# wliverno/GauNEGF

Measured on AMD Instinct MI355X. Metric: energy-points/sec (complex128 G(E) solves), higher is better.
Workload: dtype f64 (complex128)

## Files before the change

gaunegf_amd/csrc/chain_rs_inverse.h:

```cpp
#pragma once
#include "negf_common.h"
#include "wave_utils.h"

namespace {

constexpr int RS_THREADS = 256;
constexpr int RS_WAVES = 4;
#ifndef RS_PANEL
#define RS_PANEL 8
#endif
constexpr int RS_NB = RS_PANEL;
#ifndef RS_PRIO
#define RS_PRIO 1
#endif
#ifndef RS_REMAINDER
#define RS_REMAINDER 1
#endif
#ifndef RS_ROW_MODE
#define RS_ROW_MODE 0
#endif
#ifndef RS_LA_FLAGS
#define RS_LA_FLAGS 0
#endif
#ifndef RS_RR
#define RS_RR 1
#endif
#ifndef RS_UPD_3M
#define RS_UPD_3M 1
#endif
#ifndef RS_HALF_STRIPS
#define RS_HALF_STRIPS 1
#endif
#ifndef RS_ABLATE
#define RS_ABLATE 0
#endif
#ifndef RS_STAMPS
#define RS_STAMPS 0
#endif

template <int CTRL, int ROW_MASK = 0xF>
__device__ __forceinline__ unsigned rs_dpp_max_u32(unsigned k)
{
    const unsigned o = (unsigned)__builtin_amdgcn_update_dpp(0, (int)k, CTRL, ROW_MASK, 0xF, true);
    return o > k ? o : k;
}

__device__ __forceinline__ unsigned rs_wave_max_u32(unsigned k)
{
    k = rs_dpp_max_u32<0xB1>(k);
    k = rs_dpp_max_u32<0x4E>(k);
    k = rs_dpp_max_u32<0x141>(k);
    k = rs_dpp_max_u32<0x140>(k);
    k = rs_dpp_max_u32<0x142, 0xA>(k);
    k = rs_dpp_max_u32<0x143, 0xC>(k);
    return (unsigned)__builtin_amdgcn_readlane((int)k, 63);
}

__device__ __forceinline__ void zmfma4(double& ar, double& ai, cplx pa, cplx qb)
{
    ar = __builtin_amdgcn_mfma_f64_4x4x4f64(pa.x, qb.x, ar, 0, 0, 0);
    ar = __builtin_amdgcn_mfma_f64_4x4x4f64(pa.y, -qb.y, ar, 0, 0, 0);
    ai = __builtin_amdgcn_mfma_f64_4x4x4f64(pa.x, qb.y, ai, 0, 0, 0);
    ai = __builtin_amdgcn_mfma_f64_4x4x4f64(pa.y, qb.x, ai, 0, 0, 0);
}
__device__ __forceinline__ void zmfma4_conjb(double& ar, double& ai, cplx pa, cplx b)
{
    ar = __builtin_amdgcn_mfma_f64_4x4x4f64(pa.x, b.x, ar, 0, 0, 0);
// ... 4 lines not shown
#define RS_M3S(A, B, C, PR, PI, PS, QR, QI, QS) do { double a_ = (A)[0], b_ = (B)[0], c_ = (C)[0]; mfma3s(a_, b_, c_, PR, PI, PS, QR, QI, QS); (A)[0] = a_; (B)[0] = b_; (C)[0] = c_; } while (0)
#define RS_ZMFMA4(ACCR, ACCI, PA, QB) do { double r_ = (ACCR)[0], i_ = (ACCI)[0]; zmfma4(r_, i_, PA, QB); (ACCR)[0] = r_; (ACCI)[0] = i_; } while (0)
#define RS_ZMFMA4C(ACCR, ACCI, PA, QB) do { double r_ = (ACCR)[0], i_ = (ACCI)[0]; zmfma4_conjb(r_, i_, PA, QB); (ACCR)[0] = r_; (ACCI)[0] = i_; } while (0)

__device__ __forceinline__ void mfma3(d4& a, d4& b, d4& c, double pr, double pi, double ps, double qr, double qi, double qs)
{
    a = __builtin_amdgcn_mfma_f64_16x16x4f64(pr, qr, a, 0, 0, 0);
    b = __builtin_amdgcn_mfma_f64_16x16x4f64(pi, qi, b, 0, 0, 0);
    c = __builtin_amdgcn_mfma_f64_16x16x4f64(ps, qs, c, 0, 0, 0);
}
#ifndef RS_3M_GEMM
#define RS_3M_GEMM 1
#endif
__device__ __forceinline__ void mfma3s(double& a, double& b, double& c, double pr, double pi, double ps, double qr, double qi, double qs)
{
    a = __builtin_amdgcn_mfma_f64_4x4x4f64(pr, qr, a, 0, 0, 0);
    b = __builtin_amdgcn_mfma_f64_4x4x4f64(pi, qi, b, 0, 0, 0);
    c = __builtin_amdgcn_mfma_f64_4x4x4f64(ps, qs, c, 0, 0, 0);
}

template <class T>
__device__ __forceinline__ T rs_opaque(T v)
{
    asm volatile("" : "+v"(v));
    return v;
}

__device__ __forceinline__ double rs_readlane_f64(double v, int srclane)
{
    return __hiloint2double(__builtin_amdgcn_readlane(__double2hiint(v), srclane),
                            __builtin_amdgcn_readlane(__double2loint(v), srclane));
}

template <int P>
__device__ __forceinline__ void rs_factor(int n, cplx* W, int* pivrow, int* colof, cplx* rowline ,
                                          int p0, int pw, int lane, unsigned long long* fst = nullptr )
{
    const int r = rs_opaque(lane);
    cplx a[RS_NB];
    bool avail = r < n && colof[r] < 0;
    cplx myip = cmake(1.0, 0.0);
    cplx* wrow = W + r * P + p0;
#pragma unroll
    for (int s = 0; s < RS_NB; ++s) {
        const cplx v = wrow[s];
        const bool ok = (r < n) & (s < pw);
        a[s] = cmake(ok ? v.x : 0.0, ok ? v.y : 0.0);
    }
#pragma unroll
    for (int j = 0; j < RS_NB; ++j) {
        if (j < pw) {
            const bool stamp_here = fst && j == 4;
            unsigned long long tq0 = 0, tq1 = 0, tq2 = 0, tq3 = 0, tq4 = 0;
            if (stamp_here) tq0 = __builtin_amdgcn_s_memtime();
            const double v = cabs1(a[j]);
            const unsigned hi = (avail && v == v) ? (unsigned)__double2hiint(v) : 0u;
            const unsigned m = rs_wave_max_u32(hi);
            int pphys;
            if (m != 0) {
                pphys = (int)__ffsll((unsigned long long)__ballot(hi == m)) - 1;
            } else {
                const unsigned long long av = __ballot(avail);
                pphys = av ? (int)__ffsll(av) - 1 : 0x7fffffff;
            }
            pphys = __builtin_amdgcn_readfirstlane(pphys);
            if (stamp_here) tq1 = __builtin_amdgcn_s_memtime();
            const bool is_piv = r == pphys;
            cplx rb[RS_NB];
#if RS_ROW_MODE == 0
            __builtin_amdgcn_wave_barrier();
            if (is_piv) {
                pivrow[p0 + j] = pphys; colof[pphys] = p0 + j;
#pragma unroll
                for (int s = 0; s < RS_NB; ++s) rowline[s] = a[s];
            }
            __builtin_amdgcn_fence(__ATOMIC_RELEASE, "wavefront");
            __builtin_amdgcn_wave_barrier();
            __builtin_amdgcn_fence(__ATOMIC_ACQUIRE, "wavefront");
#pragma unroll
            for (int s = 0; s < RS_NB; ++s) rb[s] = rowline[s];
#elif RS_ROW_MODE == 1
            if (is_piv) { pivrow[p0 + j] = pphys; colof[pphys] = p0 + j; }
#pragma unroll
            for (int s = 0; s < RS_NB; ++s)
                rb[s] = cmake(rs_readlane_f64(a[s].x, pphys), rs_readlane_f64(a[s].y, pphys));
#else
            if (is_piv) { pivrow[p0 + j] = pphys; colof[pphys] = p0 + j; }
            const int baddr = pphys << 2;
#pragma unroll
            for (int s = 0; s < RS_NB; ++s) {
                rb[s].x = __hiloint2double(__builtin_amdgcn_ds_bpermute(baddr, __double2hiint(a[s].x)),
                                           __builtin_amdgcn_ds_bpermute(baddr, __double2loint(a[s].x)));
                rb[s].y = __hiloint2double(__builtin_amdgcn_ds_bpermute(baddr, __double2hiint(a[s].y)),
                                           __builtin_amdgcn_ds_bpermute(baddr, __double2loint(a[s].y)));
            }
#endif
            if (stamp_here) { asm volatile("s_waitcnt lgkmcnt(0)" ::: "memory"); tq2 = __builtin_amdgcn_s_memtime(); }
            const cplx pv = rb[j];
            const double d = pv.x * pv.x + pv.y * pv.y;
            double sc = __builtin_amdgcn_rcp(d);
            sc = fma(sc, fma(-d, sc, 1.0), sc);
            sc = fma(sc, fma(-d, sc, 1.0), sc);
            const cplx ip = cmake(pv.x * sc, -pv.y * sc);
            const cplx mf = cneg(cmul(a[j], ip));
            const cplx coef = cmake(is_piv ? 0.0 : mf.x, is_piv ? 0.0 : mf.y);
            if (stamp_here) { asm volatile("" :: "v"(coef.x), "v"(coef.y)); tq3 = __builtin_amdgcn_s_memtime(); }
#pragma unroll
            for (int s = 0; s < RS_NB; ++s) a[s] = cfma(a[s], coef, rb[s]);
            if (stamp_here) {
#pragma unroll
                for (int s = 0; s < RS_NB; ++s) asm volatile("" :: "v"(a[s].x), "v"(a[s].y));
                tq4 = __builtin_amdgcn_s_memtime();
                if (lane == 0) { fst[0] = tq0; fst[1] = tq1; fst[2] = tq2; fst[3] = tq3; fst[4] = tq4; }
            }
            a[j] = is_piv ? cmake(1.0, 0.0) : coef;
            myip = cmake(is_piv ? ip.x : myip.x, is_piv ? ip.y : myip.y);
            avail = avail && !is_piv;
        }
    }
    if (r < n) {
#pragma unroll
        for (int s = 0; s < RS_NB; ++s)
            if (s < pw) {
                wrow[s] = cmul(a[s], myip);
            }
    }
}

template <int P, int NKS, int TR >
__device__ __forceinline__ void rs_load_qf(const cplx* W, const int* pivrow, int tj, int p0, int pw, int fi, int fk,
                                           cplx (&qf)[NKS])
{
    const int col = (TR >= 0 && tj == TR) ? TR * 16 + (fi & 3) : tj * 16 + fi;
#pragma unroll
    for (int ks = 0; ks < NKS; ++ks) {
        const int k = ks * 4 + fk;
        const cplx v = W[pivrow[p0 + k] * P + col];
        const bool ok = k < pw;
        qf[ks] = cmake(ok ? v.x : 0.0, ok ? v.y : 0.0);
    }
}

__device__ __forceinline__ void rs_wait_count(const unsigned* cnt, unsigned target)
{
    while (*reinterpret_cast<const volatile unsigned*>(cnt) < target) __builtin_amdgcn_s_sleep(1);
}

template <int P, int NKS, int TR>
__device__ __forceinline__ void rs_zero_pivot_rows(int n, cplx* W, const int* pivrow, int tj, int p0, int pw, int fi, int fk,
                                                   int clo, int chi)
{
    const int col = (TR >= 0 && tj == TR) ? TR * 16 + (fi & 3) : tj * 16 + fi;
    if (col >= clo && col < chi && col < n) {
#pragma unroll
        for (int ks = 0; ks < NKS; ++ks) {
            const int k = ks * 4 + fk;
            if (k < pw) W[pivrow[p0 + k] * P + col] = cmake(0.0, 0.0);
        }
    }
}

template <int P, int NKS, int TR, bool MASK >
__device__ __forceinline__ void rs_update_tile(int n, cplx* W, const int* colof, int ti, int tj, int p0, int pw,
                                               int fi, int fk, const cplx (&qf)[NKS], int clo, int chi ,
                                               const unsigned* wait_cnt = nullptr, unsigned wait_target = 0 )
{
    const bool rowstrip = TR >= 0 && ti == TR, colstrip = TR >= 0 && tj == TR;
    if (!rowstrip && !colstrip) {
        cplx* cbase = W + (ti * 16 + fk) * P + tj * 16 + fi;
        const cplx* pbase = W + (ti * 16 + fi) * P + p0 + fk;
        cplx cv[4], pa[NKS];
// ... 14 lines not shown
            if (M3) mfma3(ua, ub, uc, pa[ks].x, pa[ks].y, pa[ks].x + pa[ks].y, qf[ks].x, qf[ks].y, qf[ks].x + qf[ks].y);
            else zmfma(ua, uc, pa[ks], qf[ks]);
        }
        if (wait_cnt) rs_wait_count(wait_cnt, wait_target);
#pragma unroll
        for (int r = 0; r < 4; ++r) {
            const int i = ti * 16 + fk + 4 * r;
            const int cj = tj * 16 + fi;
            if (i < n && cj < n && cj >= clo && cj < chi) cbase[4 * r * P] = M3 ? cmake(ua[r] - ub[r], uc[r] - ua[r] - ub[r]) : cmake(ua[r], uc[r]);
        }
    } else {
        const int row = rowstrip ? TR * 16 + fk : ti * 16 + 4 * (fi >> 2) + fk;
        const int col = colstrip ? TR * 16 + (fi & 3) : tj * 16 + fi;
        const bool mine = !(rowstrip && colstrip) || (fi >> 2) == 0;
        const cplx* prow = W + (rowstrip ? TR * 16 + (fi & 3) : ti * 16 + fi) * P + p0 + fk;
        cplx* cptr = W + row * P + col;
        const int cf = MASK ? colof[row] : -1;
        const cplx cv = *cptr;
        cplx pa[NKS];
#pragma unroll
        for (int ks = 0; ks < NKS; ++ks) pa[ks] = prow[ks * 4];
        const bool keep = !MASK || !(cf >= p0 && cf < p0 + pw);
        double ua = keep ? cv.x : 0.0, ub = 0.0, uc = keep ? cv.x + cv.y : 0.0;
#pragma unroll
        for (int ks = 0; ks < NKS; ++ks)
            mfma3s(ua, ub, uc, pa[ks].x, pa[ks].y, pa[ks].x + pa[ks].y, qf[ks].x, qf[ks].y, qf[ks].x + qf[ks].y);
        if (wait_cnt) rs_wait_count(wait_cnt, wait_target);
        if (mine && row < n && col < n && col >= clo && col < chi) *cptr = cmake(ua - ub, uc - ua - ub);
    }
}

constexpr bool rs_half_strips(int nks) { return RS_HALF_STRIPS && RS_NB == 8 && nks == RS_NB / 4; }

template <int P, int NKS>
__device__ __forceinline__ void rs_load_qh(const cplx* W, const int* pivrow, int c0, int p0, int pw, int fi, int fk,
                                           cplx (&qh)[2][NKS])
{
    const int col = c0 + (fi & 3);
#pragma unroll
    for (int ks = 0; ks < NKS; ++ks) {
        const int k = ks * 4 + fk;
        const cplx* q = W + pivrow[p0 + k] * P + col;
        const cplx v0 = q[0], v1 = q[4];
        const bool ok = k < pw;
        qh[0][ks] = cmake(ok ? v0.x : 0.0, ok ? v0.y : 0.0);
        qh[1][ks] = cmake(ok ? v1.x : 0.0, ok ? v1.y : 0.0);
    }
}

template <int P, int NKS>
__device__ __forceinline__ void rs_half_mma(cplx (&cv)[2], const cplx (&pa)[NKS], const cplx (&qh)[2][NKS], const double (&qs)[2][NKS])
{
    constexpr bool M3 = RS_UPD_3M && P > 35;
    if (M3) {
        double ua[2], ub[2] = {0.0, 0.0}, uc[2];
#pragma unroll
        for (int s = 0; s < 2; ++s) { ua[s] = cv[s].x; uc[s] = cv[s].x + cv[s].y; }
#pragma unroll
        for (int ks = 0; ks < NKS; ++ks) {
            const double ps = pa[ks].x + pa[ks].y;
#pragma unroll
            for (int s = 0; s < 2; ++s) mfma3s(ua[s], ub[s], uc[s], pa[ks].x, pa[ks].y, ps, qh[s][ks].x, qh[s][ks].y, qs[s][ks]);
        }
#pragma unroll
        for (int s = 0; s < 2; ++s) cv[s] = cmake(ua[s] - ub[s], uc[s] - ua[s] - ub[s]);
    } else {
#pragma unroll
        for (int ks = 0; ks < NKS; ++ks)
#pragma unroll
            for (int s = 0; s < 2; ++s) zmfma4(cv[s].x, cv[s].y, pa[ks], qh[s][ks]);
    }
}

template <int P, int NKS, bool FULLROWS , bool MASK>
__device__ __forceinline__ void rs_update_half(int n, cplx* W, const int* colof, int ti, int p0, int pw, int fi, int fk,
                                               const cplx (&qh)[2][NKS], int c0)
{
// ... 140 lines not shown
#pragma unroll 1
            for (int tj = 0; tj < ntiles; ++tj) {
                int clo = tj * 16, chi = tj * 16 + 16;
                if (tj == tp) {
                    if (RS_NB == 16) continue;
                    if (p0 & 8) chi = p0; else clo = p0 + RS_NB;
                }
                if (has_next && tj == tl) {
                    if (RS_NB == 16) continue;
                    if (n0 & 8) chi = min(chi, n0); else clo = max(clo, n0 + RS_NB);
                }
                if (clo >= chi || clo >= n) continue;
                const bool mine = (!has_next || wave != fw) && (cnt % team == me);
                ++cnt;
                if (mine && !(RS_ABLATE & 2)) {
                    if (pw <= 4) rs_update_col<T16, P, 1, TR>(n, W, pivrow, colof, tj, p0, pw, lane, clo, chi);
                    else rs_update_col<T16, P, RS_NB / 4, TR>(n, W, pivrow, colof, tj, p0, pw, lane, clo, chi);
                }
            }
        }
        if (has_next && wave == fw) {
            if (st && lane == 0) st[16 + 2 * (sgi + 1)] = __builtin_amdgcn_s_memrealtime();
            if (RS_PRIO) __builtin_amdgcn_s_setprio(3);
            if (!(RS_ABLATE & 1)) rs_factor<P>(n, W, pivrow, colof, rowline, n0, nw, lane, (st && sgi + 1 == 1) ? st + 40 : nullptr);
            else if (lane < nw) { pivrow[n0 + lane] = n0 + lane; colof[n0 + lane] = n0 + lane; }
            if (RS_PRIO) __builtin_amdgcn_s_setprio(0);
            if (st && lane == 0) st[17 + 2 * (sgi + 1)] = __builtin_amdgcn_s_memrealtime();
        }
        stamp();
        __syncthreads();
    }
}

}
```

gaunegf_amd/csrc/k_chain1d_rs.hip:

```cpp
#include "negf_common.h"
#include "chain_mix_map.h"
#include "chain_rs_inverse.h"
#include <algorithm>
#include <type_traits>

#ifndef RS_PAD_LEADS
#define RS_PAD_LEADS 1
#endif
#ifndef RS_BATCH_MSTORE
#define RS_BATCH_MSTORE 1
#endif
#ifndef RS_MSTORE_AHEAD
#define RS_MSTORE_AHEAD 0
#endif
#ifndef RS_DENSE_MIX
#define RS_DENSE_MIX 1
#endif

namespace {

struct ChainRsArgs {
    const cplx *alpha, *Salpha, *beta, *Sbeta, *tau, *Stau;
    const cplx* pad;
    const int* nc;
// ... 53 lines not shown
    if (i == 0) { q->head = 0u; q->tail = jobs; q->jobs = jobs; q->cap = cap; }
}

__device__ __forceinline__ double rs_uniform(double v)
{
    return __hiloint2double(__builtin_amdgcn_readfirstlane(__double2hiint(v)), __builtin_amdgcn_readfirstlane(__double2loint(v)));
}
typedef double rs_d2 __attribute__((ext_vector_type(2)));
__device__ __forceinline__ unsigned long long rs_scalar_base(const void* p)
{
    unsigned long long b = reinterpret_cast<unsigned long long>(p);
    asm volatile("" : "+s"(b));
    return b;
}
__device__ __forceinline__ unsigned long long rs_scalar_advance(unsigned long long b, long long bytes)
{
    b += (unsigned long long)bytes;
    asm volatile("" : "+s"(b));
    return b;
}
__device__ __forceinline__ cplx rs_gload(unsigned long long base, unsigned const_bytes, unsigned lane_bytes)
{
    const __attribute__((address_space(1))) char* p = reinterpret_cast<const __attribute__((address_space(1))) char*>(base) + const_bytes;
    const rs_d2 v = *reinterpret_cast<const __attribute__((address_space(1))) rs_d2*>(p + lane_bytes);
    return cmake(v.x, v.y);
}
__device__ __forceinline__ void rs_gstore(unsigned long long base, unsigned const_bytes, unsigned lane_bytes, cplx v)
{
    __attribute__((address_space(1))) char* p = reinterpret_cast<__attribute__((address_space(1))) char*>(base) + const_bytes;
    rs_d2 w; w.x = v.x; w.y = v.y;
    *reinterpret_cast<__attribute__((address_space(1))) rs_d2*>(p + lane_bytes) = w;
}

template <int P, int OCC, bool GOLD_GLOBAL, bool RR>
__global__ __launch_bounds__(RS_THREADS, OCC) void chain1d_rs_kernel(
    ChainRsArgs a, const cplx* __restrict__ E, cplx* __restrict__ blk, int* __restrict__ iters,
    int* __restrict__ converged)
{
    constexpr int T16 = (P - 1 + 15) / 16;
    constexpr int KS = (P + 3) / 4 < 4 * T16 ? (P + 3) / 4 : 4 * T16;
    constexpr int WELEMS = 16 * T16 * P + 16;
    constexpr int TR = T16 - 1;
    constexpr bool REM = RS_REMAINDER && T16 >= 2 && P - 16 * TR <= 4;
    constexpr int FT = REM ? TR : T16;
    constexpr bool M3G = T16 >= 3;
    extern __shared__ __attribute__((aligned(16))) unsigned char smem_raw[];
    __shared__ int flags[2 * RS_WAVES];
    __shared__ int pivrow[64], colof[64];
    __shared__ cplx rowline[RS_NB];
    __shared__ unsigned la_cnt[2];
    unsigned la_epoch = 0;
    if (threadIdx.x == 0) { la_cnt[0] = 0u; la_cnt[1] = 0u; }

    const int slot = blockIdx.y * gridDim.x + blockIdx.x;
    constexpr bool rr = RS_RR && RR;
    __shared__ long long rr_msg;
    cplx* Ws = reinterpret_cast<cplx*>(smem_raw);
    const int tid = threadIdx.x, lane = tid & 63;
    int wave = tid >> 6;
    bool chain_roles = false;
    if (a.simd_roles) {
        unsigned hwid;
        asm volatile("s_getreg_b32 %0, hwreg(HW_REG_HW_ID)" : "=s"(hwid));
        const int simd = (hwid >> 4) & 3;
        if (lane == 0) flags[wave] = simd;
        __syncthreads();
        const int seen = (1 << flags[0]) | (1 << flags[1]) | (1 << flags[2]) | (1 << flags[3]);
        chain_roles = __builtin_amdgcn_readfirstlane(seen) == 15;
        if (chain_roles) wave = simd == 0 ? RS_WAVES - 1 : simd - 1;
// ... 358 lines not shown
            }
        }
        if (resume) {
            __syncthreads();
            if (RS_DENSE_MIX) resume_old_dense();
            else {
                const int fi = rs_opaque(lane & 15), fk = rs_opaque(lane >> 4);
                const int col = wave * 16 + fi;
                cplx* gl = rs_opaque(gold_l);
                cplx* gg = GOLD_GLOBAL ? rs_opaque(gold_g) : nullptr;
#pragma unroll
                for (int ks = 0; ks < KS; ++ks) {
                    if (ks < ksteps && col < n && ks * 4 + fk < n) {
                        const cplx v = Ws[(ks * 4 + fk) * P + col];
                        if (!GOLD_GLOBAL || ks < LS_CT || (ks == LS_CT && lds_slots > LS_CT)) gl[ks * 4 * n] = v; else gg[ks * RS_THREADS] = v;
                    }
                }
            }
        }
        if (tid < 64) { colof[tid] = -1; pivrow[tid] = 0; }
        __syncthreads();
        return true;
    };

    bool need_job = true;
    while (true) {
        if (__builtin_expect(need_job, 0)) {
            if (!next_job()) break;
            need_job = false;
        }
        unsigned long long* st = (RS_STAMPS && a.stamps && job == 0 && count == a.stamp_sweep) ? a.stamps : nullptr;
        if (st && tid == 0) st[0] = __builtin_amdgcn_s_memrealtime();
        if (!gc_hit && !skip) {
            rs_inverse<T16, P, REM ? TR : -1>(n, Ws, pivrow, colof, rowline, tid, wave, chain_roles, la_cnt, la_epoch, st ? st + 8 : nullptr);
            if (st && tid == 0) st[1] = __builtin_amdgcn_s_memrealtime();
            if (!(RS_ABLATE & 8) || first) { if (RS_DENSE_MIX) gather_mix_dense(first, st); else gather_mix(first, st); }
            else { if (tid < 64) colof[tid] = -1; __syncthreads(); }
            if (st && tid == 0) st[2] = __builtin_amdgcn_s_memrealtime();
            if (!first) ++count;
            first = false;
        }
        if (__builtin_expect(skip, 0)) {
            skip = false;
        } else if (gc_hit || (a.force_iters >= 0 ? count >= a.force_iters : !(over && count < a.max_iter))) {
            final_pass = true;
            opS = Stau; opM = tau; opz = e;
            if (a.gc_mode == 1) {
                cplx* gcj = a.gcache + (size_t)b * a.blk_stride + off;
                for (int t = tid; t < n * n; t += RS_THREADS) { const int i = t / n; gcj[t] = Ws[i * P + (t - i * n)]; }
            }
        } else if (__builtin_expect(rr && count >= q_end, 0)) {
            if (tid == 0) rr_msg = rs_rr_waiting(a.rr_q) ? 1 : 0;
            __syncthreads();
            const bool sw = rr_msg != 0;
            __syncthreads();
            if (sw) {
                cplx* gsj = blk + (size_t)b * a.blk_stride + off;
                for (int t = tid; t < n * n; t += RS_THREADS) { const int i = t / n; gsj[t] = Ws[i * P + (t - i * n)]; }
                __threadfence();
                __syncthreads();
                if (tid == 0) rs_rr_push(a.rr_q, job, count);
                need_job = true;
                continue;
            }
            q_end = count + a.rr_quantum;
        }
// ... 62 lines not shown
#pragma unroll
                for (int ti = 0; ti < T16; ++ti) {
                    if (RS_MSTORE_AHEAD && ti + 1 < T16) load_a(ti + 1, as[(ti + 1) & 1], aa[(ti + 1) & 1]);
                    __builtin_amdgcn_sched_barrier(0);
                    const cplx (&s)[4] = as[RS_MSTORE_AHEAD ? ti & 1 : 0];
                    const cplx (&m)[4] = aa[RS_MSTORE_AHEAD ? ti & 1 : 0];
#pragma unroll
                    for (int r = 0; r < nel(ti); ++r) {
                        const double re = mr[ti][r], im = mi[ti][r];
                        const cplx av = csub(cmul(z, s[r]), m[r]);
                        const int i = rowc(ti, r) + (smap(ti) ? lis : fks), j = smap(ti) ? ljs : ljn;
                        const bool ok = !REM ? (i < n && j < n) : ((ti < TR || i < n) && (!SC || j < n));
                        if (ok) (smap(ti) ? wsc : wn)[rowc(ti, r) * P] = cmake(av.x - re, av.y - im);
                    }
                    __builtin_amdgcn_sched_barrier(0);
                    if (!RS_MSTORE_AHEAD && ti + 1 < T16) load_a(ti + 1, as[0], aa[0]);
                }
            };
            if (!REM || wave < TR) mstore(std::false_type{});
            else if (wave == TR) mstore(std::true_type{});
        } else {
#pragma unroll
            for (int ti = 0; ti < T16; ++ti) {
                for_tile(ti, wave, mr[ti], mi[ti], mc[ti], true, fis, fks, [&](int r, int i, int j, double re, double im) {
                    const cplx av = Aat(i, j);
                    if (i < n && j < n) Ws[i * P + j] = cmake(av.x - re, av.y - im);
                });
                __builtin_amdgcn_sched_barrier(0);
            }
        }
        __syncthreads();
        if (st && tid == 0) st[4] = __builtin_amdgcn_s_memrealtime();
    }
}

}

bool chain1d_lds_supported(int nc_max) { return nc_max <= 64; }

namespace {
int rs_rr_quantum(int user)
{
    if (user >= 0) return user;
    static int q = -1;
    if (q < 0) { const char* e = getenv("NEGF_CHAIN_RR"); q = e ? std::max(atoi(e), 0) : 100; }
    return q;
}
size_t rs_gold_elems(int nc_max, int n_contacts, int nb)
{
    return (size_t)rs_mix_reserved_slots(nc_max) * RS_THREADS * n_contacts * nb;
}
size_t rs_ring_entries(int n_contacts, int nb, int max_sweeps, int rr_user)
{
    const int q = rs_rr_quantum(rr_user);
    if (q <= 0 || max_sweeps <= q) return 0;
    const size_t jobs = (size_t)n_contacts * nb;
    const size_t cap = jobs * ((size_t)max_sweeps / q + 1) + 2048;
    return (cap >> 27) ? 0 : cap;
}
}

size_t chain1d_lds_scratch_elems(int nc_max, int n_contacts, int nb, int max_sweeps, int rr_quantum)
{
    return rs_gold_elems(nc_max, n_contacts, nb) + 1 + (rs_ring_entries(n_contacts, nb, max_sweeps, rr_quantum) + 1) / 2;
}

// ... 7 lines not shown
    const size_t wmat = (size_t)(16 * T16 * P + 16) * sizeof(cplx);
    const size_t gold_lds = (size_t)n_max * n_max * sizeof(cplx);
    auto fits = [](size_t smem, int per_cu) { return ((smem + 832 + 1279) / 1280) * 1280 * per_cu <= 160 * 1024; };
    ChainRsArgs al = a; al.gold_lds_off = 16 * T16 * P + 16; al.gold_lds_slots = 1 << 20;
    ChainRsArgs ag = a; ag.gold_lds_off = (n_max + 2) * P;
    constexpr int LS_FIT = (16 * T16 * P + 16 - (P + 2) * P) / (4 * P);
    ag.gold_lds_slots = std::min(std::max(0, (16 * T16 * P + 16 - ag.gold_lds_off) / (4 * n_max)), std::max(LS_FIT, 0) + 1);
    if (ag.gold_lds_slots < std::max(LS_FIT, 0)) ag.gold_lds_slots = 0;
    static int n_cus = 0;
    if (!n_cus) {
        int dev = 0; hipDeviceProp_t prop;
        n_cus = (hipGetDevice(&dev) == hipSuccess && hipGetDeviceProperties(&prop, dev) == hipSuccess) ? prop.multiProcessorCount : 256;
    }
    auto launch = [&](auto kern, auto kern_rr, size_t smem, int occ) {
        ChainRsArgs aa = smem > wmat ? al : ag;
        dim3 grid(n_contacts, nb);
        const int jobs = n_contacts * nb, slots = rr_slots > 0 ? std::min(rr_slots, occ * n_cus) : occ * n_cus;
        const bool rr = RS_RR && aa.rr_quantum > 0 && jobs > slots && (aa.order == nullptr || rr_forced);
        if (rr) {
            hipLaunchKernelGGL(rs_rr_init_kernel, dim3((rr_cap + 255) / 256), dim3(256), 0, st, aa.rr_q, rr_cap, (unsigned)jobs);
            grid = dim3(slots, 1);
        } else aa.rr_quantum = 0;
        static int log_env = -1;
        if (log_env < 0) log_env = getenv("NEGF_CHAIN_LOG") ? 1 : 0;
        if (log_env) fprintf(stderr, "[chain launch] jobs %d slots %d quantum %d order %d gc_mode %d\n", jobs, slots, aa.rr_quantum, aa.order ? 1 : 0, aa.gc_mode);
        auto go = [&](auto k) {
            if (hipFuncSetAttribute(reinterpret_cast<const void*>(k), hipFuncAttributeMaxDynamicSharedMemorySize, 140 * 1024) != hipSuccess)
                (void)hipGetLastError();
            hipLaunchKernelGGL(k, grid, dim3(RS_THREADS), smem, st, aa, E, blk, iters, conv);
        };
        if (rr) go(kern_rr); else go(kern);
    };
    constexpr int OCC_MAX = T16 <= 2 ? 4 : 3;
    if (occ_env != 2 && fits(wmat + gold_lds, OCC_MAX)) launch(chain1d_rs_kernel<P, OCC_MAX, false, false>, chain1d_rs_kernel<P, OCC_MAX, false, true>, wmat + gold_lds, OCC_MAX);
    else if (occ_env != 2 && gold_scratch && fits(wmat, OCC_MAX)) launch(chain1d_rs_kernel<P, OCC_MAX, true, false>, chain1d_rs_kernel<P, OCC_MAX, true, true>, wmat, OCC_MAX);
    else if (fits(wmat + gold_lds, 2) || !gold_scratch) launch(chain1d_rs_kernel<P, 2, false, false>, chain1d_rs_kernel<P, 2, false, true>, wmat + gold_lds, 2);
    else launch(chain1d_rs_kernel<P, 2, true, false>, chain1d_rs_kernel<P, 2, true, true>, wmat, 2);
}

}

void launch_chain1d_lds(hipStream_t st, const SigmaProvider& p, const int* d_nc, const int* d_blk_off, int nb,
                        const cplx* E, cplx* blk, int* iters, int* conv, cplx* gold_scratch, const int* order,
                        cplx* gcache, int gc_mode, int rr_quantum, int rr_slots, bool order_trusted)
{
    ChainRsArgs a;
    a.order = order;
    a.gcache = gcache; a.gc_mode = gcache ? gc_mode : 0;
    a.alpha = p.d_alpha; a.Salpha = p.d_Salpha; a.beta = p.d_beta; a.Sbeta = p.d_Sbeta;
    a.tau = p.d_tau; a.Stau = p.d_Stau; a.pad = p.d_lead_pad;
    a.nc = d_nc; a.blk_off = d_blk_off;
    a.n_contacts = p.n_contacts; a.blk_stride = p.blk_stride;
    a.eta = p.eta; a.conv = p.conv; a.relFactor = p.relFactor;
    a.max_iter = p.max_iter; a.force_iters = p.force_iters;
    a.gold = gold_scratch;
    a.rr_quantum = 0; a.rr_q = nullptr;
    unsigned rr_cap = 0;
    {
        const size_t cap = rs_ring_entries(p.n_contacts, nb, std::max(p.max_iter, p.force_iters), rr_quantum);
        if (gold_scratch && cap && a.gc_mode != 2) {
            a.rr_q = reinterpret_cast<RsQueue*>(gold_scratch + rs_gold_elems(p.nc_max, p.n_contacts, nb));
            rr_cap = (unsigned)cap; a.rr_quantum = rs_rr_quantum(rr_quantum);
        }
    }
    static unsigned long long* d_stamps = nullptr;
    static int want_stamps = -1;
// ... 54 lines not shown
```

Baseline: 3169.

## Add compile-time stage schedule for remainder-strip inverse with factor overlap

Adds a constexpr job schedule that packs each panel stage's trailing-update work (whole tiles, half tiles, remainder strips) into per-wave bitfields. A new rs_inverse_sched path lets three waves run those jobs while the last wave factors the next panel at raised priority. rs_factor and the q-loaders gain a FULL template flag that drops the pw masking for full-width panels. The scheduled kernel is only used for small remainder-strip sizes and only when simd_roles is set; otherwise a non-scheduled twin kernel is launched, which adds code size and template instances.

Result: faster. 3378 (median of 6 runs) (+6.6%).

```diff
diff --git a/gaunegf_amd/csrc/chain_rs_inverse.h b/gaunegf_amd/csrc/chain_rs_inverse.h
--- a/gaunegf_amd/csrc/chain_rs_inverse.h
+++ b/gaunegf_amd/csrc/chain_rs_inverse.h
@@ -1,6 +1,7 @@
 #pragma once
 #include "negf_common.h"
 #include "wave_utils.h"
+#include "chain_rs_sched.h"
 
 namespace {
 
@@ -33,6 +34,12 @@
 #endif
 #ifndef RS_ABLATE
 #define RS_ABLATE 0
+#endif
+#ifndef RS_STAGE_SCHED
+#define RS_STAGE_SCHED 1
+#endif
+#ifndef RS_SCHED_FACTOR
+#define RS_SCHED_FACTOR 0
 #endif
 #ifndef RS_STAMPS
 #define RS_STAMPS 0
@@ -103,24 +110,27 @@
                             __builtin_amdgcn_readlane(__double2loint(v), srclane));
 }
 
-template <int P>
+template <int P, int NBW = RS_NB, bool FULL = false>
 __device__ __forceinline__ void rs_factor(int n, cplx* W, int* pivrow, int* colof, cplx* rowline ,
                                           int p0, int pw, int lane, unsigned long long* fst = nullptr )
 {
     const int r = rs_opaque(lane);
-    cplx a[RS_NB];
+    cplx a[NBW];
+    constexpr bool ROWSEL = !FULL || 16 * ((P - 1 + 15) / 16) < 64;
     bool avail = r < n && colof[r] < 0;
     cplx myip = cmake(1.0, 0.0);
     cplx* wrow = W + r * P + p0;
 #pragma unroll
-    for (int s = 0; s < RS_NB; ++s) {
-        const cplx v = wrow[s];
-        const bool ok = (r < n) & (s < pw);
-        a[s] = cmake(ok ? v.x : 0.0, ok ? v.y : 0.0);
-    }
-#pragma unroll
-    for (int j = 0; j < RS_NB; ++j) {
-        if (j < pw) {
+    for (int s = 0; s < NBW; ++s) {
+        if (ROWSEL) {
+            const cplx v = wrow[s];
+            const bool ok = (r < n) & (FULL || s < pw);
+            a[s] = cmake(ok ? v.x : 0.0, ok ? v.y : 0.0);
+        } else a[s] = wrow[s];
+    }
+#pragma unroll
+    for (int j = 0; j < NBW; ++j) {
+        if (FULL || j < pw) {
             const bool stamp_here = fst && j == 4;
             unsigned long long tq0 = 0, tq1 = 0, tq2 = 0, tq3 = 0, tq4 = 0;
             if (stamp_here) tq0 = __builtin_amdgcn_s_memtime();
@@ -137,29 +147,29 @@
             pphys = __builtin_amdgcn_readfirstlane(pphys);
             if (stamp_here) tq1 = __builtin_amdgcn_s_memtime();
             const bool is_piv = r == pphys;
-            cplx rb[RS_NB];
+            cplx rb[NBW];
 #if RS_ROW_MODE == 0
             __builtin_amdgcn_wave_barrier();
             if (is_piv) {
                 pivrow[p0 + j] = pphys; colof[pphys] = p0 + j;
 #pragma unroll
-                for (int s = 0; s < RS_NB; ++s) rowline[s] = a[s];
+                for (int s = 0; s < NBW; ++s) rowline[s] = a[s];
             }
             __builtin_amdgcn_fence(__ATOMIC_RELEASE, "wavefront");
             __builtin_amdgcn_wave_barrier();
             __builtin_amdgcn_fence(__ATOMIC_ACQUIRE, "wavefront");
 #pragma unroll
-            for (int s = 0; s < RS_NB; ++s) rb[s] = rowline[s];
+            for (int s = 0; s < NBW; ++s) rb[s] = rowline[s];
 #elif RS_ROW_MODE == 1
             if (is_piv) { pivrow[p0 + j] = pphys; colof[pphys] = p0 + j; }
 #pragma unroll
-            for (int s = 0; s < RS_NB; ++s)
+            for (int s = 0; s < NBW; ++s)
                 rb[s] = cmake(rs_readlane_f64(a[s].x, pphys), rs_readlane_f64(a[s].y, pphys));
 #else
             if (is_piv) { pivrow[p0 + j] = pphys; colof[pphys] = p0 + j; }
             const int baddr = pphys << 2;
 #pragma unroll
-            for (int s = 0; s < RS_NB; ++s) {
+            for (int s = 0; s < NBW; ++s) {
                 rb[s].x = __hiloint2double(__builtin_amdgcn_ds_bpermute(baddr, __double2hiint(a[s].x)),
                                            __builtin_amdgcn_ds_bpermute(baddr, __double2loint(a[s].x)));
                 rb[s].y = __hiloint2double(__builtin_amdgcn_ds_bpermute(baddr, __double2hiint(a[s].y)),
@@ -177,10 +187,10 @@
             const cplx coef = cmake(is_piv ? 0.0 : mf.x, is_piv ? 0.0 : mf.y);
             if (stamp_here) { asm volatile("" :: "v"(coef.x), "v"(coef.y)); tq3 = __builtin_amdgcn_s_memtime(); }
 #pragma unroll
-            for (int s = 0; s < RS_NB; ++s) a[s] = cfma(a[s], coef, rb[s]);
+            for (int s = 0; s < NBW; ++s) a[s] = cfma(a[s], coef, rb[s]);
             if (stamp_here) {
 #pragma unroll
-                for (int s = 0; s < RS_NB; ++s) asm volatile("" :: "v"(a[s].x), "v"(a[s].y));
+                for (int s = 0; s < NBW; ++s) asm volatile("" :: "v"(a[s].x), "v"(a[s].y));
                 tq4 = __builtin_amdgcn_s_memtime();
                 if (lane == 0) { fst[0] = tq0; fst[1] = tq1; fst[2] = tq2; fst[3] = tq3; fst[4] = tq4; }
             }
@@ -191,14 +201,14 @@
     }
     if (r < n) {
 #pragma unroll
-        for (int s = 0; s < RS_NB; ++s)
-            if (s < pw) {
+        for (int s = 0; s < NBW; ++s)
+            if (FULL || s < pw) {
                 wrow[s] = cmul(a[s], myip);
             }
     }
 }
 
-template <int P, int NKS, int TR >
+template <int P, int NKS, int TR , bool FULL = false >
 __device__ __forceinline__ void rs_load_qf(const cplx* W, const int* pivrow, int tj, int p0, int pw, int fi, int fk,
                                            cplx (&qf)[NKS])
 {
@@ -207,7 +217,7 @@
     for (int ks = 0; ks < NKS; ++ks) {
         const int k = ks * 4 + fk;
         const cplx v = W[pivrow[p0 + k] * P + col];
-        const bool ok = k < pw;
+        const bool ok = FULL || k < pw;
         qf[ks] = cmake(ok ? v.x : 0.0, ok ? v.y : 0.0);
     }
 }
@@ -288,7 +298,7 @@
 
 constexpr bool rs_half_strips(int nks) { return RS_HALF_STRIPS && RS_NB == 8 && nks == RS_NB / 4; }
 
-template <int P, int NKS>
+template <int P, int NKS, bool FULL = false>
 __device__ __forceinline__ void rs_load_qh(const cplx* W, const int* pivrow, int c0, int p0, int pw, int fi, int fk,
                                            cplx (&qh)[2][NKS])
 {
@@ -298,7 +308,7 @@
         const int k = ks * 4 + fk;
         const cplx* q = W + pivrow[p0 + k] * P + col;
         const cplx v0 = q[0], v1 = q[4];
-        const bool ok = k < pw;
+        const bool ok = FULL || k < pw;
         qh[0][ks] = cmake(ok ? v0.x : 0.0, ok ? v0.y : 0.0);
         qh[1][ks] = cmake(ok ? v1.x : 0.0, ok ? v1.y : 0.0);
     }
@@ -505,4 +515,189 @@
     }
 }
 
-}
+constexpr bool rs_stage_sched(int TR) { return RS_STAGE_SCHED && TR >= 2 && TR <= 3 && RS_NB == 8 && RS_HALF_STRIPS && !RS_LA_FLAGS && !RS_ABLATE; }
+
+template <int P, int NKS, int TR, bool MASK, bool RANGE>
+__device__ __forceinline__ void rs_rowstrip_tile(int n, cplx* W, const int* colof, int tj, int p0, int fi, int fk,
+                                                 const cplx (&qf)[NKS], int clo)
+{
+    const int row = TR * 16 + fk, col = tj * 16 + fi;
+    const cplx* prow = W + (TR * 16 + (fi & 3)) * P + p0 + fk;
+    cplx* cptr = W + row * P + col;
+    const int cf = MASK ? colof[row] : -1;
+    const cplx cv = *cptr;
+    cplx pa[NKS];
+#pragma unroll
+    for (int ks = 0; ks < NKS; ++ks) pa[ks] = prow[ks * 4];
+    const bool keep = !MASK || !(cf >= p0 && cf < p0 + 4 * NKS);
+    double ua = keep ? cv.x : 0.0, ub = 0.0, uc = keep ? cv.x + cv.y : 0.0;
+#pragma unroll
+    for (int ks = 0; ks < NKS; ++ks)
+        mfma3s(ua, ub, uc, pa[ks].x, pa[ks].y, pa[ks].x + pa[ks].y, qf[ks].x, qf[ks].y, qf[ks].x + qf[ks].y);
+    if (row < n && (!RANGE || (unsigned)(col - clo) < 8u)) *cptr = cmake(ua - ub, uc - ua - ub);
+}
+
+template <int P, int NKS>
+__device__ __forceinline__ void rs_zero_pivot_rows_full(cplx* W, const int* pivrow, int p0, int fk, int col)
+{
+#pragma unroll
+    for (int ks = 0; ks < NKS; ++ks) W[pivrow[p0 + ks * 4 + fk] * P + col] = cmake(0.0, 0.0);
+}
+template <int P>
+__device__ __forceinline__ void rs_zero_pivot_rows_narrow(cplx* W, const int* pivrow, int p0, int pw, int fk, int col)
+{
+    double z = 0.0;
+    asm volatile("" : "+v"(z));
+    if (fk < pw) W[pivrow[p0 + fk] * P + col] = cmake(z, z);
+}
+
+template <int P, int TR, int NKS, bool FULL>
+__device__ __forceinline__ void rs_job_whole(int n, cplx* W, const int* pivrow, const int* colof, int tj, int p0, int pw, int lane)
+{
+    const int fi = rs_opaque(lane & 15), fk = rs_opaque(lane >> 4);
+    const int col = tj * 16 + fi;
+    cplx qf[NKS];
+    rs_load_qf<P, NKS, -1, FULL>(W, pivrow, tj, p0, pw, fi, fk, qf);
+    if (FULL) rs_zero_pivot_rows_full<P, NKS>(W, pivrow, p0, fk, col);
+    else rs_zero_pivot_rows_narrow<P>(W, pivrow, p0, pw, fk, col);
+    constexpr bool M3 = RS_UPD_3M && P > 35;
+    double qs[NKS];
+#pragma unroll
+    for (int ks = 0; ks < NKS; ++ks) qs[ks] = qf[ks].x + qf[ks].y;
+    cplx* cbase = W + fk * P + col;
+    const cplx* pbase = W + fi * P + p0 + fk;
+    cplx cv[2][4], pa[2][NKS];
+    auto fetch = [&](int ti, int s) __attribute__((always_inline)) {
+#pragma unroll
+        for (int r = 0; r < 4; ++r) cv[s][r] = cbase[(ti * 16 + 4 * r) * P];
+#pragma unroll
+        for (int ks = 0; ks < NKS; ++ks) pa[s][ks] = pbase[ti * 16 * P + ks * 4];
+    };
+    fetch(0, 0);
+#pragma unroll
+    for (int ti = 0; ti < TR; ++ti) {
+        const int s = ti & 1;
+        if (ti + 1 < TR) fetch(ti + 1, s ^ 1);
+        d4 ua, ub = {0, 0, 0, 0}, uc;
+#pragma unroll
+        for (int r = 0; r < 4; ++r) { ua[r] = cv[s][r].x; uc[r] = M3 ? cv[s][r].x + cv[s][r].y : cv[s][r].y; }
+#pragma unroll
+        for (int ks = 0; ks < NKS; ++ks) {
+            if (M3) mfma3(ua, ub, uc, pa[s][ks].x, pa[s][ks].y, pa[s][ks].x + pa[s][ks].y, qf[ks].x, qf[ks].y, qs[ks]);
+            else zmfma(ua, uc, pa[s][ks], qf[ks]);
+        }
+#pragma unroll
+        for (int r = 0; r < 4; ++r) cbase[(ti * 16 + 4 * r) * P] = M3 ? cmake(ua[r] - ub[r], uc[r] - ua[r] - ub[r]) : cmake(ua[r], uc[r]);
+        __builtin_amdgcn_sched_barrier(0);
+    }
+    rs_rowstrip_tile<P, NKS, TR, false, false>(n, W, colof, tj, p0, fi, fk, qf, 0);
+}
+
+template <int P, int TR>
+__device__ __forceinline__ void rs_job_half(int n, cplx* W, const int* pivrow, const int* colof, int tj, int clo, int p0, int lane)
+{
+    constexpr int NKS = RS_NB / 4;
+    const int fi = rs_opaque(lane & 15), fk = rs_opaque(lane >> 4);
+    cplx qf[NKS], qh[2][NKS];
+    double qs[2][NKS];
+    rs_load_qf<P, NKS, -1, true>(W, pivrow, tj, p0, RS_NB, fi, fk, qf);
+    rs_load_qh<P, NKS, true>(W, pivrow, clo, p0, RS_NB, fi, fk, qh);
+    if ((unsigned)(tj * 16 + fi - clo) < 8u) rs_zero_pivot_rows_full<P, NKS>(W, pivrow, p0, fk, tj * 16 + fi);
+#pragma unroll
+    for (int ks = 0; ks < NKS; ++ks) { qs[0][ks] = qh[0][ks].x + qh[0][ks].y; qs[1][ks] = qh[1][ks].x + qh[1][ks].y; }
+    const int row = 4 * (fi >> 2) + fk;
+    cplx* cbase = W + row * P + clo + (fi & 3);
+    const cplx* pbase = W + fi * P + p0 + fk;
+    cplx cv[2][2], pa[2][NKS];
+    auto fetch = [&](int ti, int s) __attribute__((always_inline)) {
+        cv[s][0] = cbase[ti * 16 * P]; cv[s][1] = cbase[ti * 16 * P + 4];
+#pragma unroll
+        for (int ks = 0; ks < NKS; ++ks) pa[s][ks] = pbase[ti * 16 * P + ks * 4];
+    };
+    fetch(0, 0);
+#pragma unroll
+    for (int ti = 0; ti < TR; ++ti) {
+        const int s = ti & 1;
+        if (ti + 1 < TR) fetch(ti + 1, s ^ 1);
+        rs_half_mma<P, NKS>(cv[s], pa[s], qh, qs);
+        cbase[ti * 16 * P] = cv[s][0]; cbase[ti * 16 * P + 4] = cv[s][1];
+        __builtin_amdgcn_sched_barrier(0);
+    }
+    rs_rowstrip_tile<P, NKS, TR, false, true>(n, W, colof, tj, p0, fi, fk, qf, clo);
+}
+
+template <int T16, int P, int TR>
+__device__ __forceinline__ void rs_job_strip(int n, cplx* W, const int* pivrow, const int* colof, int p0, int lane)
+{
+    constexpr int NKS = RS_NB / 4;
+    const int fi = rs_opaque(lane & 15), fk = rs_opaque(lane >> 4);
+    const int col = TR * 16 + (fi & 3);
+    cplx qf[NKS];
+    rs_load_qf<P, NKS, TR, true>(W, pivrow, TR, p0, RS_NB, fi, fk, qf);
+    if (col < n) rs_zero_pivot_rows_full<P, NKS>(W, pivrow, p0, fk, col);
+#pragma unroll
+    for (int ti = 0; ti < T16; ++ti) {
+        rs_update_tile<P, NKS, TR, false>(n, W, colof, ti, TR, p0, RS_NB, fi, fk, qf, TR * 16, TR * 16 + 16);
+        __builtin_amdgcn_sched_barrier(0);
+    }
+}
+
+template <int T16, int P, int TR>
+__device__ __forceinline__ void rs_inverse_sched(int n, cplx* W, int* pivrow, int* colof, cplx* rowline, int tid, int wave,
+                                                 unsigned long long* st = nullptr)
+{
+    static_assert(TR == T16 - 1 && rs_sched_fits(TR), "a remainder-strip class");
+    constexpr int NKS = RS_NB / 4;
+    const int lane = tid & 63;
+    int sti = 0;
+    auto stamp = [&]() __attribute__((always_inline)) { if (st && tid == 0) st[sti] = __builtin_amdgcn_s_memrealtime(); ++sti; };
+    wave = __builtin_amdgcn_readfirstlane(wave);
+    const unsigned long long jobs = wave == 0 ? rs_sched_word(TR, 0) : wave == 1 ? rs_sched_word(TR, 1) : wave == 2 ? rs_sched_word(TR, 2) : 0ull;
+#pragma unroll 1
+    for (int sgi = -1; sgi < 2 * TR; ++sgi) {
+        const int p0 = sgi * RS_NB, n0 = p0 + RS_NB;
+        const bool full_next = sgi + 1 < 2 * TR;
+        if (sgi >= 0) {
+            const int fi = rs_opaque(lane & 15), fk = rs_opaque(lane >> 4);
+            const int tl = n0 >> 4;
+            cplx qh[2][NKS];
+            cplx (&qf)[NKS] = qh[0];
+            if (full_next) {
+                if (wave < TR) rs_load_qh<P, NKS, true>(W, pivrow, n0, p0, RS_NB, fi, fk, qh);
+                else if (wave == TR) rs_load_qf<P, NKS, -1, true>(W, pivrow, tl, p0, RS_NB, fi, fk, qf);
+            } else if (wave < T16) rs_load_qf<P, NKS, TR, true>(W, pivrow, TR, p0, RS_NB, fi, fk, qf);
+            __syncthreads();
+            if (full_next) {
+                if (wave < TR) rs_update_half<P, NKS, true, true>(n, W, colof, wave, p0, RS_NB, fi, fk, qh, n0);
+                else if (wave == TR) rs_rowstrip_tile<P, NKS, TR, true, true>(n, W, colof, tl, p0, fi, fk, qf, n0);
+            } else if (wave < T16) rs_update_tile<P, NKS, TR, true>(n, W, colof, wave, TR, p0, RS_NB, fi, fk, qf, n0, n0 + RS_NB);
+            __syncthreads();
+            unsigned c = (unsigned)(jobs >> (RS_STAGE_BITS * sgi)) & ((1u << RS_STAGE_BITS) - 1u);
+#pragma unroll 1
+            while (c) {
+                const unsigned kind = c & 3u;
+                const int tj = (int)(c >> 2) & 3;
+                if (kind == RS_JOB_WHOLE) rs_job_whole<P, TR, NKS, true>(n, W, pivrow, colof, tj, p0, RS_NB, lane);
+                else if (kind == RS_JOB_HALF) rs_job_half<P, TR>(n, W, pivrow, colof, tj, tj * 16 + (int)((c >> 4) & 1u) * 8, p0, lane);
+                else rs_job_strip<T16, P, TR>(n, W, pivrow, colof, p0, lane);
+                c >>= RS_JOB_BITS;
+            }
+        }
+        if (wave == RS_WAVES - 1) {
+            if (st && lane == 0) st[16 + 2 * (sgi + 1)] = __builtin_amdgcn_s_memrealtime();
+            if (RS_PRIO) __builtin_amdgcn_s_setprio(3);
+            if (!RS_SCHED_FACTOR) rs_factor<P>(n, W, pivrow, colof, rowline, n0, full_next ? RS_NB : n - n0, lane, (st && sgi + 1 == 1) ? st + 40 : nullptr);
+            else if (full_next) rs_factor<P, RS_NB, true>(n, W, pivrow, colof, rowline, n0, RS_NB, lane, (st && sgi + 1 == 1) ? st + 40 : nullptr);
+            else rs_factor<P, 4, false>(n, W, pivrow, colof, rowline, n0, n - n0, lane);
+            if (RS_PRIO) __builtin_amdgcn_s_setprio(0);
+            if (st && lane == 0) st[17 + 2 * (sgi + 1)] = __builtin_amdgcn_s_memrealtime();
+        }
+        stamp();
+        __syncthreads();
+    }
+    if (wave < TR) rs_job_whole<P, TR, 1, false>(n, W, pivrow, colof, wave, TR * 16, n - TR * 16, lane);
+    stamp();
+    __syncthreads();
+}
+
+}
diff --git a/gaunegf_amd/csrc/chain_rs_sched.h b/gaunegf_amd/csrc/chain_rs_sched.h
--- /dev/null
+++ b/gaunegf_amd/csrc/chain_rs_sched.h
@@ -0,0 +1,58 @@
+#pragma once
+
+#if defined(__HIPCC__) || defined(__CUDACC__)
+#define RS_SCHED_HD __host__ __device__
+#else
+#define RS_SCHED_HD
+#endif
+
+constexpr unsigned RS_JOB_NONE = 0;
+constexpr unsigned RS_JOB_WHOLE = 1;
+constexpr unsigned RS_JOB_HALF = 2;
+constexpr unsigned RS_JOB_STRIP = 3;
+constexpr int RS_JOB_BITS = 5, RS_STAGE_BITS = 10;
+constexpr int RS_SCHED_TEAM = 3;
+
+RS_SCHED_HD constexpr unsigned rs_sched_job(int TR, int sgi, int idx)
+{
+    const int tp = sgi >> 1, odd = sgi & 1, tl = tp + odd;
+    int cnt = 0;
+    for (int tj = 0; tj <= TR; ++tj) {
+        unsigned code = RS_JOB_NONE;
+        if (!odd) {
+            if (tj == tp) continue;
+            code = (tj == TR ? RS_JOB_STRIP : RS_JOB_WHOLE) | (unsigned)tj << 2;
+        } else if (tj == tp) {
+            code = RS_JOB_HALF | (unsigned)tj << 2;
+        } else if (tj == tl) {
+            if (tl == TR) continue;
+            code = RS_JOB_HALF | (unsigned)tj << 2 | 1u << 4;
+        } else {
+            code = (tj == TR ? RS_JOB_STRIP : RS_JOB_WHOLE) | (unsigned)tj << 2;
+        }
+        if (cnt++ == idx) return code;
+    }
+    return RS_JOB_NONE;
+}
+
+RS_SCHED_HD constexpr unsigned long long rs_sched_word(int TR, int role)
+{
+    unsigned long long w = 0;
+    for (int sgi = 0; sgi < 2 * TR; ++sgi) {
+        const unsigned long long st = rs_sched_job(TR, sgi, role) | (unsigned long long)rs_sched_job(TR, sgi, role + RS_SCHED_TEAM) << RS_JOB_BITS;
+        w |= st << (RS_STAGE_BITS * sgi);
+    }
+    return w;
+}
+
+RS_SCHED_HD constexpr bool rs_sched_fits(int TR)
+{
+    if (TR < 1 || 2 * TR * RS_STAGE_BITS > 64) return false;
+    for (int sgi = 0; sgi < 2 * TR; ++sgi) {
+        if (rs_sched_job(TR, sgi, 2 * RS_SCHED_TEAM) != RS_JOB_NONE) return false;
+        for (int role = 0; role < RS_SCHED_TEAM; ++role)
+            if (rs_sched_job(TR, sgi, role) == RS_JOB_NONE && rs_sched_job(TR, sgi, role + RS_SCHED_TEAM) != RS_JOB_NONE) return false;
+    }
+    return true;
+}
+static_assert(rs_sched_fits(1) && rs_sched_fits(2) && rs_sched_fits(3), "stage schedule of the strip classes");
diff --git a/gaunegf_amd/csrc/k_chain1d_rs.hip b/gaunegf_amd/csrc/k_chain1d_rs.hip
--- a/gaunegf_amd/csrc/k_chain1d_rs.hip
+++ b/gaunegf_amd/csrc/k_chain1d_rs.hip
@@ -109,9 +109,9 @@
     *reinterpret_cast<__attribute__((address_space(1))) rs_d2*>(p + lane_bytes) = w;
 }
 
-template <int P, int OCC, bool GOLD_GLOBAL, bool RR>
-__global__ __launch_bounds__(RS_THREADS, OCC) void chain1d_rs_kernel(
-    ChainRsArgs a, const cplx* __restrict__ E, cplx* __restrict__ blk, int* __restrict__ iters,
+template <int P, int OCC, bool GOLD_GLOBAL, bool RR, bool SCHED>
+__device__ __forceinline__ void chain1d_rs_body(
+    const ChainRsArgs& a, const cplx* __restrict__ E, cplx* __restrict__ blk, int* __restrict__ iters,
     int* __restrict__ converged)
 {
     constexpr int T16 = (P - 1 + 15) / 16;
@@ -536,6 +536,8 @@
         unsigned long long* st = (RS_STAMPS && a.stamps && job == 0 && count == a.stamp_sweep) ? a.stamps : nullptr;
         if (st && tid == 0) st[0] = __builtin_amdgcn_s_memrealtime();
         if (!gc_hit && !skip) {
+            if constexpr (SCHED && REM && rs_stage_sched(REM ? TR : -1)) rs_inverse_sched<T16, P, TR>(n, Ws, pivrow, colof, rowline, tid, wave, st ? st + 8 : nullptr);
+            else
             rs_inverse<T16, P, REM ? TR : -1>(n, Ws, pivrow, colof, rowline, tid, wave, chain_roles, la_cnt, la_epoch, st ? st + 8 : nullptr);
             if (st && tid == 0) st[1] = __builtin_amdgcn_s_memrealtime();
             if (!(RS_ABLATE & 8) || first) { if (RS_DENSE_MIX) gather_mix_dense(first, st); else gather_mix(first, st); }
@@ -664,6 +666,22 @@
         __syncthreads();
         if (st && tid == 0) st[4] = __builtin_amdgcn_s_memrealtime();
     }
+}
+
+template <int P, int OCC, bool GOLD_GLOBAL, bool RR>
+__global__ __launch_bounds__(RS_THREADS, OCC) void chain1d_rs_kernel(
+    ChainRsArgs a, const cplx* __restrict__ E, cplx* __restrict__ blk, int* __restrict__ iters,
+    int* __restrict__ converged)
+{
+    chain1d_rs_body<P, OCC, GOLD_GLOBAL, RR, true>(a, E, blk, iters, converged);
+}
+
+template <int P, int OCC, bool GOLD_GLOBAL, bool RR>
+__global__ __launch_bounds__(RS_THREADS, OCC) void chain1d_rs_wn_kernel(
+    ChainRsArgs a, const cplx* __restrict__ E, cplx* __restrict__ blk, int* __restrict__ iters,
+    int* __restrict__ converged)
+{
+    chain1d_rs_body<P, OCC, GOLD_GLOBAL, RR, false>(a, E, blk, iters, converged);
 }
 
 }
@@ -737,6 +755,16 @@
         if (rr) go(kern_rr); else go(kern);
     };
     constexpr int OCC_MAX = T16 <= 2 ? 4 : 3;
+    constexpr bool STRIPS = RS_REMAINDER && T16 >= 2 && P - 16 * (T16 - 1) <= 4;
+    if constexpr (STRIPS && rs_stage_sched(T16 - 1)) {
+        if (!a.simd_roles) {
+            if (occ_env != 2 && fits(wmat + gold_lds, OCC_MAX)) launch(chain1d_rs_wn_kernel<P, OCC_MAX, false, false>, chain1d_rs_wn_kernel<P, OCC_MAX, false, true>, wmat + gold_lds, OCC_MAX);
+            else if (occ_env != 2 && gold_scratch && fits(wmat, OCC_MAX)) launch(chain1d_rs_wn_kernel<P, OCC_MAX, true, false>, chain1d_rs_wn_kernel<P, OCC_MAX, true, true>, wmat, OCC_MAX);
+            else if (fits(wmat + gold_lds, 2) || !gold_scratch) launch(chain1d_rs_wn_kernel<P, 2, false, false>, chain1d_rs_wn_kernel<P, 2, false, true>, wmat + gold_lds, 2);
+            else launch(chain1d_rs_wn_kernel<P, 2, true, false>, chain1d_rs_wn_kernel<P, 2, true, true>, wmat, 2);
+            return;
+        }
+    }
     if (occ_env != 2 && fits(wmat + gold_lds, OCC_MAX)) launch(chain1d_rs_kernel<P, OCC_MAX, false, false>, chain1d_rs_kernel<P, OCC_MAX, false, true>, wmat + gold_lds, OCC_MAX);
     else if (occ_env != 2 && gold_scratch && fits(wmat, OCC_MAX)) launch(chain1d_rs_kernel<P, OCC_MAX, true, false>, chain1d_rs_kernel<P, OCC_MAX, true, true>, wmat, OCC_MAX);
     else if (fits(wmat + gold_lds, 2) || !gold_scratch) launch(chain1d_rs_kernel<P, 2, false, false>, chain1d_rs_kernel<P, 2, false, true>, wmat + gold_lds, 2);
```
